# Corleno/Nonstationary_Multivariate_Gaussian_Process

Measured on AMD Instinct MI355X. Metric: log-posterior evals/sec (N=2048, D=3 nonseparable GP), higher is better.
Workload: dtype f64

## Files before the change

### nonstationary_multivariate_gaussian_process_amd/csrc/nmgp_chol.hip

```cpp
#include "nmgp_internal.h"
#include <cstring>

namespace nmgpk {

static inline int cdiv_c(long long a, long long b) { return (int)((a + b - 1) / b); }

typedef double v4d __attribute__((ext_vector_type(4)));

#define SY_BM 128
#define SY_BK 16
#define SY_LD (SY_BM + 16)
#define SY_SB 8

__device__ __forceinline__ int clamp_row_pair(int r, int rows) {
    int rc = r < rows - 1 ? r : rows - 2;
    return rc < 0 ? 0 : rc;
}

__device__ __forceinline__ double fast_recip(double p) {
    double x = __builtin_amdgcn_rcp(p);
    double e = fma(-p, x, 1.0);
    x = fma(x, e, x);
    e = fma(-p, x, 1.0);
    x = fma(x, e, x);
    return x;
}

template <int KC, int GC>
__device__ __forceinline__ void potf2_step(double (&a)[16], double (*colbuf)[64], double* pivs, int nb,
                                           int* __restrict__ info, int goff, int r, int g, int tid) {
    constexpr int c = 4 * KC + GC;
    constexpr int NKC = (GC == 3) ? KC + 1 : KC;
    constexpr int NGC = (GC == 3) ? 0 : GC + 1;
    if (c >= nb) return;
    const double* cb = colbuf[c & 1];
    const double piv = cb[c];
    const double mine = cb[r];
    double t[16];
#pragma unroll
    for (int kk = KC; kk < 16; ++kk) t[kk] = cb[4 * kk + g];
    if (tid == 0) {
        pivs[c] = piv;
        if (!(piv > 0.0)) atomicCAS(info, 0, goff + c + 1);
    }
    const double pinv = fast_recip(piv);
    const double f = mine * pinv;
    if (c + 1 < 64) {
        if (NKC < 16) {
            const int cc = 4 * NKC + g;
            const double upd = fma(-f, t[NKC < 16 ? NKC : 15], a[NKC < 16 ? NKC : 15]);
            const bool on = (g == NGC) && (cc <= r);
            if (NKC < 16) a[NKC < 16 ? NKC : 15] = on ? upd : a[NKC < 16 ? NKC : 15];
            if (g == NGC) colbuf[(c + 1) & 1][r] = a[NKC < 16 ? NKC : 15];
        }
        __syncthreads();
    }
#pragma unroll
    for (int kk = KC; kk < 16; ++kk) {
        const int cc = 4 * kk + g;
        const double upd = fma(-f, t[kk], a[kk]);
        bool on = (kk > KC || g > GC) && (cc <= r);
        if (kk == NKC) on = on && (g != NGC);
        a[kk] = on ? upd : a[kk];
    }
}

template <int KC>
__device__ __forceinline__ void potf2_steps4(double (&a)[16], double (*colbuf)[64], double* pivs, int nb,
                                             int* __restrict__ info, int goff, int r, int g, int tid) {
    potf2_step<KC, 0>(a, colbuf, pivs, nb, info, goff, r, g, tid);
    potf2_step<KC, 1>(a, colbuf, pivs, nb, info, goff, r, g, tid);
    potf2_step<KC, 2>(a, colbuf, pivs, nb, info, goff, r, g, tid);
    potf2_step<KC, 3>(a, colbuf, pivs, nb, info, goff, r, g, tid);
}

__device__ __forceinline__ void potf2_body(double* __restrict__ A, int lda, int nb, int* __restrict__ info, int goff, int tid,
                                           double (*colbuf)[64], double* pivs) {
    const int r = tid & 63, g = (tid >> 6) & 3;
    double a[16];
#pragma unroll
    for (int kk = 0; kk < 16; ++kk) {
        const int c = 4 * kk + g;
        double v = (r == c) ? 1.0 : 0.0;
        if (r < nb && c <= r) v = A[(size_t)c * lda + r];
        a[kk] = v;
    }
    if (tid < 64) pivs[tid] = 1.0;
    if (g == 0) colbuf[0][r] = a[0];
    __syncthreads();
#define PF(K) potf2_steps4<K>(a, colbuf, pivs, nb, info, goff, r, g, tid)
    PF(0); PF(1); PF(2); PF(3); PF(4); PF(5); PF(6); PF(7); PF(8); PF(9); PF(10); PF(11); PF(12); PF(13); PF(14); PF(15);
#undef PF
    __syncthreads();
#pragma unroll
    for (int kk = 0; kk < 16; ++kk) {
        const int c = 4 * kk + g;
        if (r < nb && c <= r) A[(size_t)c * lda + r] = a[kk] * rsqrt(pivs[c]);
    }
}

typedef double v2d __attribute__((ext_vector_type(2)));
typedef int v4i __attribute__((ext_vector_type(4)));

__device__ __forceinline__ void syrk_fused_first_block(double* lds, const v4d (&acc)[2][2][2], bool owner, int wj,
                                                       double* __restrict__ C, int ldc, int* __restrict__ info, int goff);

#define SY_SMEM (4 * SY_BK * SY_LD)
#define SCHUR_PATCH (32 * 33)
#define SY_SCHUR_SMEM (8 * SCHUR_PATCH + 6 * 256)
static_assert(SY_SCHUR_SMEM >= SY_SMEM && SY_SCHUR_SMEM * 8 * 2 <= 160 * 1024, "Schur epilogue LDS");

template <int M>
__device__ __forceinline__ double svc_schur_value(double sigma2, int a, int b, bool rc, const double* __restrict__ Lr, double il2,
                                                  const double* __restrict__ Lc, double kv, double nai, double gcb) {
    constexpr int UR = M <= 3 ? 8 : 1;
    const double gra = sigma2 * Lr[a * (a + 1) / 2] * il2;
    double s = 0.0;
#pragma unroll UR
    for (int q = 1; q <= b; ++q) s += Lr[a * (a + 1) / 2 + q] * Lc[b * (b + 1) / 2 + q];
    double v = kv * s;
    if (rc) v += sigma2 * ((a == b ? 1.0 : 0.0) + Lr[a * (a + 1) / 2] * Lr[b * (b + 1) / 2] * il2);
    v += gra * nai * gcb;
    return v;
}

template <int M, bool ALLB>
__device__ __forceinline__ void svc_schur_entries(const SchurEpi& e, double sigma2, int r, const double* __restrict__ Lr, double il2,
                                                  int c, double kv, double nai, const double* gc) {
    constexpr int T = M * (M + 1) / 2;
    constexpr int UR = M <= 3 ? 8 : 1;
    const size_t Ns = (size_t)e.N;
    const double* __restrict__ Lc = e.Lv + (size_t)c * T;
    const double lcc = M <= 4 ? 0.0 : Lc[0];
#pragma unroll UR
    for (int a = 1; a < M; ++a) {
#pragma unroll UR
        for (int b = 1; b <= (ALLB ? a : a - 1); ++b) {
            const double gcb = M <= 4 ? gc[b - 1] : sigma2 * Lc[b * (b + 1) / 2] / (lcc * lcc);
            e.S[((size_t)(b - 1) * Ns + c) * e.ld + ((size_t)(a - 1) * Ns + r)] =
                svc_schur_value<M>(sigma2, a, b, r == c, Lr, il2, Lc, kv, nai, gcb);
        }
    }
}

constexpr int svc_gstride(int M) { return M + 2; }

template <int M>
__device__ __forceinline__ void svc_schur_gtable(const SchurEpi& e, double* lds, int row0, int col0, int tid) {
    constexpr int T = M * (M + 1) / 2, GS = svc_gstride(M);
    if constexpr (M <= 4) {
        double* gt = lds + 8 * SCHUR_PATCH;
        if (tid < 256) {
            const int loc = tid < 128 ? col0 + tid : row0 + tid - 128;
            if (loc < e.N) {
                const double sigma2 = exp(e.tse[0]);
                const double* Lc = e.Lv + (size_t)loc * T;
                const double l00 = Lc[0];
#pragma unroll
                for (int b = 1; b < M; ++b) gt[tid * GS + b - 1] = sigma2 * Lc[b * (b + 1) / 2] / (l00 * l00);
                gt[tid * GS + M - 1] = 1.0 / (l00 * l00);
                gt[tid * GS + M] = e.x[loc];
                gt[tid * GS + M + 1] = e.ell[loc];
            }
        }
        __syncthreads();
    }
}

template <int M>
__device__ __forceinline__ void svc_schur_patch(const SchurEpi& e, double* P, const double* lds, int i0, int j0, int row0, int col0,
                                                int lane) {
    constexpr int T_ = M * (M + 1) / 2, GS = svc_gstride(M);
    constexpr int QU = M <= 3 ? 2 : 1;
    const int N = e.N;
    const size_t Ns = (size_t)N;
    const double sigma2 = exp(e.tse[0]);
    const double* gt = lds + 8 * SCHUR_PATCH;
    const int lo = lane & 31, hi = lane >> 5;
    __builtin_amdgcn_wave_barrier();
#pragma unroll
    for (int pass = 0; pass < 2; ++pass) {
        if (pass == 1 && M == 2) break;
        const int r = (pass == 0 ? i0 : j0) + lo;
        if (r < N) {
            const double* __restrict__ Lr = e.Lv + (size_t)r * T_;
            const double xr = e.x[r], lr = e.ell[r];
            const double xr2 = xr * xr, lr2 = lr * lr;
            const double l00 = Lr[0];
            const double il2 = 1.0 / (l00 * l00);
#pragma unroll QU
            for (int q = 0; q < 16; ++q) {
                const int o = 2 * q + hi;
                const int il = pass == 0 ? lo : o, jl = pass == 0 ? o : lo;
                const int c = (pass == 0 ? j0 : i0) + o;
                if (pass == 0 ? (c > r || c >= N) : (c <= r || c >= N)) continue;
                const double* gc = gt + (pass == 0 ? c - col0 : 128 + c - row0) * GS;
                if (pass == 1 && M == 3) {
                    e.S[(size_t)c * e.ld + (Ns + r)] = P[il * 33 + jl];
                    continue;
                }
                const double xc = M <= 4 ? gc[M] : e.x[c], lc = M <= 4 ? gc[M + 1] : e.ell[c];
                const double dist = (xr2 + xc * xc) - 2.0 * (xr * xc);
                const double Aa = lr2 + lc * lc;
                double kv = sqrt(2.0 * (lr * lc) / Aa) * exp(-dist / Aa);
                if (r == c) kv = NMGP_JITTER + kv;
                const double nai = P[il * 33 + jl];
                if (pass == 0) {
                    svc_schur_entries<M, true>(e, sigma2, r, Lr, il2, c, kv, nai, gc);
                    if (M == 3 && c < r) {
                        const double* Lc = e.Lv + (size_t)c * T_;
                        P[il * 33 + jl] = svc_schur_value<M>(sigma2, 2, 1, false, Lc, gc[M - 1], Lr, kv, nai, gt[(128 + r - row0) * GS]);
                    }
                } else {
                    svc_schur_entries<M, false>(e, sigma2, r, Lr, il2, c, kv, nai, gc);
                }
            }
        }
        __builtin_amdgcn_wave_barrier();
    }
}

template <int M>
__device__ __forceinline__ void svc_schur_yrow(const SchurEpi& e, int i) {
    constexpr int T = M * (M + 1) / 2;
    if (i >= e.N) return;
    const size_t Ns = (size_t)e.N;
    const int n1 = (M - 1) * e.N;
    const double sigma2 = exp(e.tse[0]);
    const double* Li = e.Lv + (size_t)i * T;
    const double l00 = Li[0];
    const double il2 = 1.0 / (l00 * l00);
    const double vi = e.y[i] / l00;
    const double r = vi - (sigma2 * il2) * e.u[i];
#pragma unroll
    for (int a = 1; a < M; ++a) e.S[((size_t)(a - 1) * Ns + i) * e.ld + n1] = e.y[(size_t)a * Ns + i] - Li[a * (a + 1) / 2] * r;
}

template <int SM = 0>
__device__ __forceinline__ void syrk_tile_fast(const double* __restrict__ A, int lda, double* __restrict__ C, int ldc, int K,
                                               int row0, int col0, bool diag, int kt0, bool beta0, int ncw, int yrow,
                                               int nyr, double* sA0, double* sB0, bool skip00 = false,
                                               int* __restrict__ finfo = nullptr, int fgoff = 0, bool mirror = false,
                                               int fresh0 = 0x7fffffff, const SchurEpi* se = nullptr) {
    constexpr int BK = 16;
    constexpr int SBUF = BK * SY_LD;
    const int tid = threadIdx.x, lane = tid & 63, w = tid >> 6;
    const int wi = w & 1, wj = w >> 1;
    const int l15 = lane & 15, l4 = lane >> 4;
    const int rp = tid & 63, cg = tid >> 6;
    const int offA = (cg * lda + row0 + 2 * rp) * 8, offB = (cg * lda + col0 + 2 * rp) * 8;
    const __amdgpu_buffer_rsrc_t rsrc = __builtin_amdgcn_make_buffer_rsrc((void*)A, 0, 0x7fffffff, 0x00020000);
    const int gstep = BK * lda * 8, ghalf = 8 * lda * 8;
    int soff = kt0 * gstep;
    const bool has_y = diag && yrow >= 0;
    const bool ywave = has_y && wi == 0 && wj >= 2;
    const int offY = ((tid & 15) * lda + yrow + (tid >> 4)) * 8;
    double* sY = sB0;
    v4i ra0, ra1, rb0, rb1;
    double ry = 0.0;
    auto gload = [&]() {
        ra0 = __builtin_amdgcn_raw_buffer_load_b128(rsrc, offA, soff, 0);
        ra1 = __builtin_amdgcn_raw_buffer_load_b128(rsrc, offA, soff + ghalf, 0);
        if (!diag) {
            rb0 = __builtin_amdgcn_raw_buffer_load_b128(rsrc, offB, soff, 0);
            rb1 = __builtin_amdgcn_raw_buffer_load_b128(rsrc, offB, soff + ghalf, 0);
        }
        if (has_y && tid < 16 * nyr) {
            typedef int v2i __attribute__((ext_vector_type(2)));
            const v2i t2 = __builtin_amdgcn_raw_buffer_load_b64(rsrc, offY, soff, 0);
            ry = __builtin_bit_cast(double, t2);
        }
        soff += gstep;
    };
    double* wA = sA0 + cg * SY_LD + 2 * rp;
    double* wB = sB0 + cg * SY_LD + 2 * rp;
    auto sstore = [&](int buf) {
        *reinterpret_cast<v4i*>(wA + buf * SBUF) = ra0;
        *reinterpret_cast<v4i*>(wA + buf * SBUF + 8 * SY_LD) = ra1;
        if (!diag) {
            *reinterpret_cast<v4i*>(wB + buf * SBUF) = rb0;
            *reinterpret_cast<v4i*>(wB + buf * SBUF + 8 * SY_LD) = rb1;
        }
        if (has_y && tid < 16 * nyr) sY[buf * 256 + tid] = ry;
    };
    const bool active = !(diag && (wi * 64 + 63 < wj * 32)) && (wj * 32 < ncw) && !(skip00 && wi == 0 && wj < 2);
    const int nk = K / BK;
    gload();
    v4d acc[2][2][2];
    if (active) {
        const int rw0 = __builtin_amdgcn_readfirstlane(row0 + wi * 64);
        const bool wload = !beta0 && rw0 < fresh0;
#pragma unroll
        for (int p = 0; p < 2; ++p) {
            const int i = row0 + wi * 64 + 32 * p + 2 * l15;
            const bool old = i < fresh0;
#pragma unroll
            for (int tj = 0; tj < 2; ++tj)
#pragma unroll
                for (int r = 0; r < 4; ++r) {
                    const int j = col0 + wj * 32 + 2 * (l4 + 4 * r) + tj;
                    double2 c = make_double2(0.0, 0.0);
                    if (wload && old) c = *reinterpret_cast<const double2*>(&C[(size_t)j * ldc + i]);
                    acc[p][0][tj][r] = -c.x;
                    acc[p][1][tj][r] = -c.y;
                }
        }
    }
    if (ywave) {
#pragma unroll
        for (int u = 0; u < 2; ++u)
#pragma unroll
            for (int t = 0; t < 2; ++t)
#pragma unroll
                for (int r = 0; r < 4; ++r) {
                    const int j = col0 + 64 * (wj - 2) + 32 * u + 2 * (l4 + 4 * r) + t;
                    acc[u][0][t][r] = (l15 < nyr && yrow + l15 < fresh0) ? -C[(size_t)j * ldc + yrow + l15] : 0.0;
                }
    }
    sstore(0);
    __syncthreads();
    const double* rA = sA0 + wi * 64 + 2 * l15 + l4 * SY_LD;
    const double* rB = (diag ? sA0 : sB0) + wj * 32 + 2 * l15 + l4 * SY_LD;
    auto compute = [&](int buf) {
        const double* tA = rA + buf * SBUF;
        const double* tB = rB + buf * SBUF;
        v2d fa[2], fb, na[2], nb;
        fa[0] = *reinterpret_cast<const v2d*>(tA);
        fa[1] = *reinterpret_cast<const v2d*>(tA + 32);
        fb = *reinterpret_cast<const v2d*>(tB);
#pragma unroll
        for (int kk = 0; kk < BK / 4; ++kk) {
            if (kk + 1 < BK / 4) {
                na[0] = *reinterpret_cast<const v2d*>(tA + (kk + 1) * 4 * SY_LD);
                na[1] = *reinterpret_cast<const v2d*>(tA + (kk + 1) * 4 * SY_LD + 32);
                nb = *reinterpret_cast<const v2d*>(tB + (kk + 1) * 4 * SY_LD);
            }
#pragma unroll
            for (int tj = 0; tj < 2; ++tj)
#pragma unroll
                for (int p = 0; p < 2; ++p)
#pragma unroll
                    for (int sx = 0; sx < 2; ++sx)
                        acc[p][sx][tj] = __builtin_amdgcn_mfma_f64_16x16x4f64(fb[tj], fa[p][sx], acc[p][sx][tj], 0, 0, 0);
            if (kk + 1 < BK / 4) {
                fa[0] = na[0];
                fa[1] = na[1];
                fb = nb;
            }
        }
    };
    const double* rY = sA0 + 64 * (wj - 2) + 2 * l15 + l4 * SY_LD;
    const int yz = (l15 < nyr) ? yrow + l15 - fresh0 - l4 : 0x7fffffff;
    auto compute_y = [&](int buf, int kb) {
        const double* tB = rY + buf * SBUF;
        const double* ty = sY + buf * 256 + l15 * 16 + l4;
#pragma unroll
        for (int kk = 0; kk < BK / 4; ++kk) {
            const v2d f0 = *reinterpret_cast<const v2d*>(tB + kk * 4 * SY_LD);
            const v2d f1 = *reinterpret_cast<const v2d*>(tB + kk * 4 * SY_LD + 32);
            const double yv = ty[4 * kk];
            const double fy = (kb + 4 * kk >= yz) ? yv : 0.0;
            acc[0][0][0] = __builtin_amdgcn_mfma_f64_16x16x4f64(f0[0], fy, acc[0][0][0], 0, 0, 0);
            acc[0][0][1] = __builtin_amdgcn_mfma_f64_16x16x4f64(f0[1], fy, acc[0][0][1], 0, 0, 0);
            acc[1][0][0] = __builtin_amdgcn_mfma_f64_16x16x4f64(f1[0], fy, acc[1][0][0], 0, 0, 0);
            acc[1][0][1] = __builtin_amdgcn_mfma_f64_16x16x4f64(f1[1], fy, acc[1][0][1], 0, 0, 0);
        }
    };
    for (int kt = kt0; kt < nk; kt += 2) {
        gload();
        if (active) compute(0);
        else if (ywave) compute_y(0, kt * BK);
        sstore(1);
        __syncthreads();
        if (kt + 2 < nk) gload();
        if (active) compute(1);
        else if (ywave) compute_y(1, kt * BK + BK);
        if (kt + 2 < nk) sstore(0);
        __syncthreads();
    }
    if constexpr (SM > 0) {
        svc_schur_gtable<SM>(*se, sA0, row0, col0, tid);
        if (active) {
            double* P = sA0 + w * SCHUR_PATCH;
#pragma unroll
            for (int p = 0; p < 2; ++p) {
#pragma unroll
                for (int sx = 0; sx < 2; ++sx)
#pragma unroll
                    for (int tj = 0; tj < 2; ++tj)
#pragma unroll
                        for (int r = 0; r < 4; ++r) P[(2 * l15 + sx) * 33 + 2 * (l4 + 4 * r) + tj] = -acc[p][sx][tj][r];
                svc_schur_patch<SM>(*se, P, sA0, row0 + wi * 64 + 32 * p, col0 + wj * 32, row0, col0, lane);
            }
        }
        if (diag && wj == 0) svc_schur_yrow<SM>(*se, row0 + wi * 64 + lane);
        return;
    }
    if (ywave && l15 < nyr) {
#pragma unroll
        for (int u = 0; u < 2; ++u)
#pragma unroll
            for (int t = 0; t < 2; ++t)
#pragma unroll
                for (int r = 0; r < 4; ++r) {
                    const int j = col0 + 64 * (wj - 2) + 32 * u + 2 * (l4 + 4 * r) + t;
                    C[(size_t)j * ldc + yrow + l15] = -acc[u][0][t][r];
                }
    }
    const bool fowner = finfo != nullptr && wi == 0 && wj < 2;
    if (active && !fowner) {
#pragma unroll
    for (int p = 0; p < 2; ++p)
#pragma unroll
        for (int tj = 0; tj < 2; ++tj)
#pragma unroll
            for (int r = 0; r < 4; ++r) {
                const int i = row0 + wi * 64 + 32 * p + 2 * l15;
                const int j = col0 + wj * 32 + 2 * (l4 + 4 * r) + tj;
                if (diag && j > i + 1) continue;
                double2 c;
                c.x = -acc[p][0][tj][r];
                c.y = -acc[p][1][tj][r];
                if (diag && j == i + 1) C[(size_t)j * ldc + i + 1] = c.y;
                else *reinterpret_cast<double2*>(&C[(size_t)j * ldc + i]) = c;
            }
    }
    if (mirror && active) {
        double* T = sA0 + w * (32 * 33);
        const int jl = lane & 31, ih = lane >> 5;
#pragma unroll
        for (int p = 0; p < 2; ++p) {
#pragma unroll
            for (int sx = 0; sx < 2; ++sx)
#pragma unroll
                for (int tj = 0; tj < 2; ++tj)
#pragma unroll
                    for (int r = 0; r < 4; ++r) T[(2 * l15 + sx) * 33 + 2 * (l4 + 4 * r) + tj] = -acc[p][sx][tj][r];
            const int rowm = col0 + wj * 32 + jl;
#pragma unroll
            for (int q = 0; q < 16; ++q) {
                const int il = 2 * q + ih;
                const int colm = row0 + wi * 64 + 32 * p + il;
                const double v = T[il * 33 + jl];
                if (colm > rowm) C[(size_t)colm * ldc + rowm] = v;
            }
        }
    }
    if (finfo != nullptr) syrk_fused_first_block(sA0, acc, fowner, wj, C, ldc, finfo, fgoff);
}

template <int NWJ, int BK, int SM = 0>
__device__ __forceinline__ void syrk_tile_body(const double* __restrict__ A, int lda, double* __restrict__ C, int ldc, int mrows,
                                               int ncols, int K, long long bstride, long long cstride, int ktri, int swz,
                                               int nbatch, int bx, int by, int bz0, double* sAb, double* sBb,
                                               int tri_row0 = 0x7fffffff, int tri_k0 = 0, int* __restrict__ finfo = nullptr,
                                               int fistride = 0, int fgoff = 0, const SchurEpi* sep = nullptr) {
    const int nyr = (ktri >> 2) & 31;
    const bool skipq = (ktri & 128) != 0;
    const bool mirror = (ktri & 512) != 0;
    const bool rowmajor = (ktri & 1024) != 0;
    const int yrow = nyr ? mrows : -1;
    (void)rowmajor;
    ktri &= 1;
    const int fresh0 = tri_row0 == 0x7fffffff ? 0x7fffffff : tri_row0 + tri_k0;
    constexpr int NT = 128 * NWJ;
    constexpr int CW = 128 / NWJ;
    constexpr int TJ = CW / 16;
    constexpr int NQ = (64 * BK) / NT;
    constexpr int CGS = NT / 64;
    double (*sA)[BK * SY_LD] = reinterpret_cast<double (*)[BK * SY_LD]>(sAb);
    double (*sB)[BK * SY_LD] = reinterpret_cast<double (*)[BK * SY_LD]>(sBb);
    int bi = bx, bj = by;
    int bz = bz0;
    if (swz) {
        const int t = bx, q = t >> 3;
        const int tiles_pm = swz > 0 ? swz : -swz;
        const long long g = swz > 0 ? ((long long)(q >> 6) * 8 + (t & 7)) * 64 + (q & 63) : (long long)t;
        int idx;
        if (finfo != nullptr) {
            if (g >= (long long)tiles_pm * nbatch) return;
            if (g < nbatch) {
                bz = (int)g;
                idx = 0;
            } else {
                const long long g2 = g - nbatch;
                bz = (int)(g2 / (tiles_pm - 1));
                idx = 1 + (int)(g2 - (long long)bz * (tiles_pm - 1));
            }
        } else {
            bz = (int)(g / tiles_pm);
            if (bz >= nbatch) return;
            idx = (int)(g - (long long)bz * tiles_pm);
        }
        const int gx = (mrows + SY_BM - 1) / SY_BM, gy = (ncols + SY_BM - 1) / SY_BM;
        if (rowmajor) {
            const int tri = gy * (gy + 1) / 2;
            if (idx < tri) {
                int b = (int)((sqrt(8.0 * (double)idx + 1.0) - 1.0) * 0.5);
                while ((b + 1) * (b + 2) / 2 <= idx) ++b;
                while (b * (b + 1) / 2 > idx) --b;
                bi = b;
                bj = idx - b * (b + 1) / 2;
            } else {
                bi = gy + (idx - tri) / gy;
                bj = (idx - tri) % gy;
            }
        } else {
        int c0 = 0, W = 0, cnt = 0;
        for (;; c0 += SY_SB) {
            W = gy - c0 < SY_SB ? gy - c0 : SY_SB;
            cnt = W * (W + 1) / 2 + (gx - c0 - W) * W;
            if (idx < cnt) break;
            idx -= cnt;
        }
        const int tri = W * (W + 1) / 2;
        if (idx < tri) {
            int b = 0;
            while (idx >= W - b) {
                idx -= W - b;
                ++b;
            }
            bj = c0 + b;
            bi = bj + idx;
        } else {
            idx -= tri;
            const int blk = idx / (SY_SB * W), in = idx - blk * (SY_SB * W);
            const int base = c0 + W + blk * SY_SB;
            const int rb = gx - base < SY_SB ? gx - base : SY_SB;
            bj = c0 + in / rb;
            bi = base + in % rb;
        }
        }
    }
    if (bi < bj) return;
    bi = __builtin_amdgcn_readfirstlane(bi);
    bj = __builtin_amdgcn_readfirstlane(bj);
    bz = __builtin_amdgcn_readfirstlane(bz);
    A += (size_t)bz * bstride;
    C += (size_t)bz * cstride;
    SchurEpi se{};
    if constexpr (SM > 0) {
        static_assert(NWJ == 4 && BK == 16, "the Schur epilogue assumes 8 waves of 64 x 32");
        constexpr int T = SM * (SM + 1) / 2;
        se = *sep;
        se.x += (size_t)(bz / se.cps) * se.xstride;
        se.y += (size_t)(bz / se.cps) * se.ystride;
        se.ell += (size_t)bz * se.N;
        se.Lv += (size_t)bz * se.N * T;
        se.tse += (size_t)bz * ((size_t)se.N * (1 + T) + 1);
        se.u += (size_t)bz * se.N;
        se.S += (size_t)bz * se.bstride;
    }
    const bool diag = (bi == bj);
    const int tid = threadIdx.x, lane = tid & 63, w = tid >> 6;
    const int wi = w & 1, wj = w >> 1;
    const int row0 = bi * SY_BM, col0 = bj * SY_BM;
    if constexpr (NWJ == 4 && BK == 16) {
        const int ncw = ncols - col0 >= SY_BM ? SY_BM : ncols - col0;
        if (row0 + SY_BM <= mrows && (ncw == SY_BM || ncw == 64) && col0 + SY_BM <= mrows && (K & 31) == 0 &&
            (long long)(K + 16) * lda * 8 < 0x7fff0000LL) {
            int kt0f = ktri ? row0 / BK : 0;
            if (row0 >= tri_row0) {
                const int z = (row0 - tri_row0 - tri_k0) / BK;
                kt0f = z > 0 ? (z & ~1) : 0;
            }
            syrk_tile_fast<SM>(A, lda, C, ldc, K, row0, col0, diag, kt0f, ktri != 0, ncw, yrow, nyr, &sA[0][0], &sB[0][0],
                               skipq && bi == 0 && bj == 0, (finfo != nullptr && bi == 0 && bj == 0) ? finfo + (size_t)bz * fistride : nullptr,
                               fgoff, mirror, fresh0, &se);
            return;
        }
    }
    const int rp = tid & 63, cg = tid >> 6;
    double2 ra[NQ], rb[NQ];

    const int ri = row0 + 2 * rp, rj = col0 + 2 * rp;
    const int ric = clamp_row_pair(ri, mrows), rjc = clamp_row_pair(rj, mrows);
    const bool ix = ri < mrows, iy = ri + 1 < mrows, jx = rj < mrows, jy = rj + 1 < mrows;
    const bool ish = ix && (ric != ri), jsh = jx && (rjc != rj);
    auto gload = [&](int k0) {
#pragma unroll
        for (int q = 0; q < NQ; ++q) {
            const int kc = k0 + cg + CGS * q;
            const double* colp = A + (size_t)(kc < K ? kc : K - 1) * lda;
            ra[q] = *reinterpret_cast<const double2*>(colp + ric);
            if (!diag) rb[q] = *reinterpret_cast<const double2*>(colp + rjc);
        }
    };
    auto sstore = [&](int buf, int k0) {
#pragma unroll
        for (int q = 0; q < NQ; ++q) {
            const int kl = cg + CGS * q;
            const bool kin = (k0 + kl) < K;
            double2 va, vb;
            va.x = (kin && ix) ? (ish ? ra[q].y : ra[q].x) : 0.0;
            va.y = (kin && iy) ? ra[q].y : 0.0;
            *reinterpret_cast<double2*>(&sA[buf][kl * SY_LD + 2 * rp]) = va;
            if (!diag) {
                vb.x = (kin && jx) ? (jsh ? rb[q].y : rb[q].x) : 0.0;
                vb.y = (kin && jy) ? rb[q].y : 0.0;
                *reinterpret_cast<double2*>(&sB[buf][kl * SY_LD + 2 * rp]) = vb;
            }
        }
    };

    const bool active = !(diag && (wi * 64 + 63 < wj * CW));
    const bool skip00g = skipq && bi == 0 && bj == 0;
    const int nk = (K + BK - 1) / BK;
    int kt0 = ktri ? (row0 / BK) : 0;
    if (row0 >= tri_row0 && row0 - tri_row0 - tri_k0 > 0) kt0 = (row0 - tri_row0 - tri_k0) / BK;
    gload(kt0 * BK);
    v4d acc[TJ][4];
#pragma unroll
    for (int tj = 0; tj < TJ; ++tj)
#pragma unroll
        for (int ti = 0; ti < 4; ++ti)
#pragma unroll
            for (int r = 0; r < 4; ++r) {
                const int i = row0 + wi * 64 + ti * 16 + (lane & 15);
                const int j = col0 + wj * CW + tj * 16 + (lane >> 4) + 4 * r;
                acc[tj][ti][r] = (!ktri && active && i < mrows && j < ncols && i >= j) ? C[(size_t)j * ldc + i] : 0.0;
            }
    if (row0 + SY_BM > fresh0) {
#pragma unroll
        for (int tj = 0; tj < TJ; ++tj)
#pragma unroll
            for (int ti = 0; ti < 4; ++ti)
#pragma unroll
                for (int r = 0; r < 4; ++r)
                    acc[tj][ti][r] = (row0 + wi * 64 + ti * 16 + (lane & 15) >= fresh0) ? 0.0 : acc[tj][ti][r];
    }
    sstore(0, kt0 * BK);
    __syncthreads();
    for (int kt = kt0; kt < nk; ++kt) {
        const int cur = (kt - kt0) & 1;
        if (kt + 1 < nk) gload((kt + 1) * BK);
        if (active) {
            const double* tA = sA[cur] + wi * 64 + (lane & 15) + (lane >> 4) * SY_LD;
            const double* tB = (diag ? sA[cur] : sB[cur]) + wj * CW + (lane & 15) + (lane >> 4) * SY_LD;
            double fa[4], fb[TJ], na[4], nb[TJ];
#pragma unroll
            for (int t = 0; t < 4; ++t) fa[t] = tA[t * 16];
#pragma unroll
            for (int t = 0; t < TJ; ++t) fb[t] = -tB[t * 16];
#pragma unroll
            for (int kk = 0; kk < BK / 4; ++kk) {
                if (kk + 1 < BK / 4) {
#pragma unroll
                    for (int t = 0; t < 4; ++t) na[t] = tA[(kk + 1) * 4 * SY_LD + t * 16];
#pragma unroll
                    for (int t = 0; t < TJ; ++t) nb[t] = -tB[(kk + 1) * 4 * SY_LD + t * 16];
                }
#pragma unroll
                for (int tj = 0; tj < TJ; ++tj)
#pragma unroll
                    for (int ti = 0; ti < 4; ++ti)
                        acc[tj][ti] = __builtin_amdgcn_mfma_f64_16x16x4f64(fb[tj], fa[ti], acc[tj][ti], 0, 0, 0);
                if (kk + 1 < BK / 4) {
#pragma unroll
                    for (int t = 0; t < 4; ++t) fa[t] = na[t];
#pragma unroll
                    for (int t = 0; t < TJ; ++t) fb[t] = nb[t];
                }
            }
        }
        if (kt + 1 < nk) sstore(cur ^ 1, (kt + 1) * BK);
        __syncthreads();
    }
    if constexpr (SM > 0) {
        svc_schur_gtable<SM>(se, sAb, row0, col0, tid);
        if (active) {
            double* P = sAb + w * SCHUR_PATCH;
#pragma unroll
            for (int h = 0; h < 2; ++h) {
#pragma unroll
                for (int tj = 0; tj < TJ; ++tj)
#pragma unroll
                    for (int t2 = 0; t2 < 2; ++t2)
#pragma unroll
                        for (int r = 0; r < 4; ++r)
                            P[(t2 * 16 + (lane & 15)) * 33 + tj * 16 + (lane >> 4) + 4 * r] = acc[tj][2 * h + t2][r];
                svc_schur_patch<SM>(se, P, sAb, row0 + wi * 64 + 32 * h, col0 + wj * CW, row0, col0, lane);
// ... 1364 lines not shown
```

Measured before the change: 1695.

## Remap Schur SYRK waves and skip zero lower-triangular k-blocks per group

For the Schur-epilogue instantiation of the SYRK tile, the wave-to-subtile mapping changes, and a specialized compute loop runs per 32-row group. Each group skips MFMA work on diagonal tiles above the diagonal and on early k-iterations where the operands are known to be zero, using compile-time group masks. It also software-prefetches the next LDS fragments. The intent is to cut wasted MFMA work on structurally zero blocks. The cost is more code specialization, and correctness depends on the assumed zero pattern of the inputs.

```diff
diff --git a/nonstationary_multivariate_gaussian_process_amd/csrc/nmgp_chol.hip b/nonstationary_multivariate_gaussian_process_amd/csrc/nmgp_chol.hip
--- a/nonstationary_multivariate_gaussian_process_amd/csrc/nmgp_chol.hip
+++ b/nonstationary_multivariate_gaussian_process_amd/csrc/nmgp_chol.hip
@@ -236,6 +236,8 @@
     for (int a = 1; a < M; ++a) e.S[((size_t)(a - 1) * Ns + i) * e.ld + n1] = e.y[(size_t)a * Ns + i] - Li[a * (a + 1) / 2] * r;
 }
 
+template <int V> struct SyIc { static constexpr int value = V; };
+
 template <int SM = 0>
 __device__ __forceinline__ void syrk_tile_fast(const double* __restrict__ A, int lda, double* __restrict__ C, int ldc, int K,
                                                int row0, int col0, bool diag, int kt0, bool beta0, int ncw, int yrow,
@@ -245,7 +247,7 @@
     constexpr int BK = 16;
     constexpr int SBUF = BK * SY_LD;
     const int tid = threadIdx.x, lane = tid & 63, w = tid >> 6;
-    const int wi = w & 1, wj = w >> 1;
+    const int wi = SM > 0 ? w >> 2 : w & 1, wj = SM > 0 ? w & 3 : w >> 1;
     const int l15 = lane & 15, l4 = lane >> 4;
     const int rp = tid & 63, cg = tid >> 6;
     const int offA = (cg * lda + row0 + 2 * rp) * 8, offB = (cg * lda + col0 + 2 * rp) * 8;
@@ -366,6 +368,60 @@
             acc[1][0][1] = __builtin_amdgcn_mfma_f64_16x16x4f64(f1[1], fy, acc[1][0][1], 0, 0, 0);
         }
     };
+    if constexpr (SM > 0) {
+        const int g0 = 2 * wi, g1 = 2 * wi + 1;
+        const bool on0 = active && !(diag && g0 < wj), on1 = active && !(diag && g1 < wj);
+        auto compute_g = [&](auto G, int buf) {
+            constexpr int g = decltype(G)::value;
+            const double* tA = rA + buf * SBUF;
+            const double* tB = rB + buf * SBUF;
+            v2d fa[2], fb, na[2], nb;
+#pragma unroll
+            for (int p = 0; p < 2; ++p)
+                if ((g >> p) & 1) fa[p] = *reinterpret_cast<const v2d*>(tA + 32 * p);
+            fb = *reinterpret_cast<const v2d*>(tB);
+#pragma unroll
+            for (int kk = 0; kk < BK / 4; ++kk) {
+                if (kk + 1 < BK / 4) {
+#pragma unroll
+                    for (int p = 0; p < 2; ++p)
+                        if ((g >> p) & 1) na[p] = *reinterpret_cast<const v2d*>(tA + (kk + 1) * 4 * SY_LD + 32 * p);
+                    nb = *reinterpret_cast<const v2d*>(tB + (kk + 1) * 4 * SY_LD);
+                }
+#pragma unroll
+                for (int tj = 0; tj < 2; ++tj)
+#pragma unroll
+                    for (int p = 0; p < 2; ++p)
+                        if ((g >> p) & 1)
+#pragma unroll
+                            for (int sx = 0; sx < 2; ++sx)
+                                acc[p][sx][tj] = __builtin_amdgcn_mfma_f64_16x16x4f64(fb[tj], fa[p][sx], acc[p][sx][tj], 0, 0, 0);
+                if (kk + 1 < BK / 4) {
+#pragma unroll
+                    for (int p = 0; p < 2; ++p)
+                        if ((g >> p) & 1) fa[p] = na[p];
+                    fb = nb;
+                }
+            }
+        };
+        auto compute_m = [&](int mode, int buf) {
+            if (mode == 3) compute_g(SyIc<3>{}, buf);
+            else if (mode == 2) compute_g(SyIc<2>{}, buf);
+            else if (mode == 1) compute_g(SyIc<1>{}, buf);
+        };
+        for (int kt = kt0; kt < nk; kt += 2) {
+            const int it = (kt - kt0) >> 1;
+            const int mode = (on0 && it >= g0 ? 1 : 0) | (on1 && it >= g1 ? 2 : 0);
+            gload();
+            compute_m(mode, 0);
+            sstore(1);
+            __syncthreads();
+            if (kt + 2 < nk) gload();
+            compute_m(mode, 1);
+            if (kt + 2 < nk) sstore(0);
+            __syncthreads();
+        }
+    } else {
     for (int kt = kt0; kt < nk; kt += 2) {
         gload();
         if (active) compute(0);
@@ -377,6 +433,7 @@
         else if (ywave) compute_y(1, kt * BK + BK);
         if (kt + 2 < nk) sstore(0);
         __syncthreads();
+    }
     }
     if constexpr (SM > 0) {
         svc_schur_gtable<SM>(*se, sA0, row0, col0, tid);
```

Result: no change. 1703 (median of 6 runs) (+0.4%).
